# ilovepose/fast-human-pose-estimation.pytorch

Hardware: AMD Instinct MI355X
Metric: images/sec FPD train step (4-stack HG student, 8-stack teacher) 256x256 (higher is better)
Workload: dtype bf16; 1 GPU; configs[1]: hourglass student S=4 F=128 + teacher S=8 F=256, 256x256, batch 32/GPU, fused FPD step incl. Adam, teacher forward one batch ahead on a 2nd stream; global_batch=32, parallelism=dp1, backend=mfma, launch=one native plan call per phase, kernels launched eagerly on 3 streams, ranks=1, finite=True

## Files before the change

### fast-human-pose-estimation.pytorch_amd/csrc/api.hip

```cpp
#include <cstdarg>
#include <cstdio>
#include <cstdlib>
#include <cstring>
#include <string>
#include <vector>

#include "common.h"

int fpd_conv_mfma_launch(const fpd_conv_t& a, hipStream_t st);
int fpd_conv_tile_launch(const fpd_conv_t& a, hipStream_t st);
int fpd_conv_pp_launch(const fpd_conv_t& a, hipStream_t st);
int fpd_conv_c1_launch(const fpd_conv_t& a, hipStream_t st);
int fpd_conv_c3_launch(const fpd_conv_t& a, hipStream_t st);
int fpd_conv_c3_pair_launch(const fpd_conv_t& a, const fpd_conv_t& b, hipStream_t st);
int fpd_conv_c3_fold_ok(const fpd_conv_t& a, const fpd_conv_t* b);
int fpd_conv_c3_option(int which, int value);
int fpd_conv_c1_pair_launch(const fpd_conv_t& a, const fpd_conv_t& b, hipStream_t st);
int fpd_conv_c1_fold_ok(const fpd_conv_t& a, const fpd_conv_t* b);
int fpd_conv_c1_option(int which, int value);
int fpd_conv_c1_wgrad_partials(const fpd_conv_t& a);
int fpd_conv_c1_pair_wgrad_partials(const fpd_conv_t& a, const fpd_conv_t& b, int* na, int* nb);
int fpd_conv_pp_pair_launch(const fpd_conv_t& a, const fpd_conv_t& b, hipStream_t st);
int fpd_conv_pp_fold_ok(const fpd_conv_t& a, const fpd_conv_t* b);
int fpd_conv_tile_fold_ok(const fpd_conv_t& a);
int fpd_conv_tile_pair_fold_ok(const fpd_conv_t& a, const fpd_conv_t& b);
int fpd_conv_pp_option(int which, int value);
int fpd_conv_pp_wgrad_partials(const fpd_conv_t& a);
int fpd_conv_pp_pair_wgrad_partials(const fpd_conv_t& a, const fpd_conv_t& b, int* na, int* nb);
int fpd_conv_tile_pair_launch(const fpd_conv_t& a, const fpd_conv_t& b, hipStream_t st);
int fpd_bneck_fused_launch(const fpd_bneck_t& a, hipStream_t st);
int fpd_bneck_fold_launch(const fpd_bneck_t& a, float* out, hipStream_t st);
int fpd_pck_launch(const fpd_pck_t& a, hipStream_t st);
int fpd_conv_smallc_launch(const fpd_conv_t& a, hipStream_t st);
bool fpd_conv_f8_domain(const fpd_conv_t& a);
int fpd_conv_tile_f8_launch(const fpd_conv_t& a, const void* w8, const float* wscale, hipStream_t st);
int fpd_weight_quant_f8_launch(const fpd_wquant_entry_t* table, int n, hipStream_t st);
int fpd_flip_w_launch(const float* x, float* y, int64_t rows, int W, hipStream_t st);
int fpd_flip_merge_launch(const fpd_flipmerge_t& p, hipStream_t st);
int fpd_final_preds_launch(const fpd_finalpreds_t& p, hipStream_t st);
int fpd_render_targets_launch(const fpd_targets_t& a, hipStream_t st);
int fpd_warp_affine_launch(const fpd_warp_t& a, hipStream_t st);
int fpd_head_fused_launch(const fpd_head_t& a, hipStream_t st);
int fpd_head_fold_launch(const fpd_head_t& a, float* out, hipStream_t st);
int fpd_bneck_fused_pair_launch(const fpd_bneck_t& a, const fpd_bneck_t& b, hipStream_t st);
int fpd_wgrad_mfma_launch(const fpd_wgrad_t& a, hipStream_t st);
int fpd_wgrad_tile_launch(const fpd_wgrad_t& a, hipStream_t st);
int fpd_wgrad_tile_partials(const fpd_wgrad_t& a);
int fpd_wgrad_smallc_launch(const fpd_wgrad_t& a, hipStream_t st);
int fpd_wgrad_smallc_partials(const fpd_wgrad_t& a);
int fpd_wgrad_mfma_partials(const fpd_wgrad_t& a);
int fpd_wgrad_naive_partials(const fpd_wgrad_t& a);
int fpd_stem_wgrad_mfma_partials(const fpd_stem_t& a);
int fpd_stem_wgrad_partials(const fpd_stem_t& a);
int fpd_wreduce_launch(const fpd_wreduce_entry_t* table, int n, int64_t max_elems, hipStream_t st);
int fpd_conv_naive_launch(const fpd_conv_t& a, hipStream_t st);
int fpd_wgrad_naive_launch(const fpd_wgrad_t& a, hipStream_t st);
int fpd_stem_forward_launch(const fpd_stem_t& a, hipStream_t st);
int fpd_stem_forward_mfma_launch(const fpd_stem_t& a, hipStream_t st);
int fpd_stem_forward_s2d_launch(const fpd_stem_t& a, hipStream_t st);
int fpd_stem_wgrad_s2d_launch(const fpd_stem_t& a, hipStream_t st);
int fpd_stem_wgrad_s2d_partials(const fpd_stem_t& a);
int fpd_stem_wgrad_mfma_launch(const fpd_stem_t& a, hipStream_t st);
int fpd_stem_wgrad_launch(const fpd_stem_t& a, hipStream_t st);
int fpd_elementwise_launch(const fpd_ew_t& a, hipStream_t st);
int fpd_elementwise_pair_launch(const fpd_ew_t& a, const fpd_ew_t& b, hipStream_t st);
int fpd_affsum_launch(const fpd_affsum_t& a, hipStream_t st);
int fpd_loss_launch(const fpd_loss_t& a, hipStream_t st);
int fpd_adam_launch(const fpd_adam_t& a, hipStream_t st);
int fpd_weight_prep_launch(const fpd_wprep_entry_t* table, int n, int64_t max_elems, int dtype, hipStream_t st);
int fpd_bn_update_running_launch(const fpd_bnupd_entry_t* table, int n, hipStream_t st);
int fpd_cast_launch(const void* src, void* dst, int64_t n, int sd, int dd, hipStream_t st);
int fpd_nchw_to_nhwc_launch(const float* src, void* dst, int N, int C, int H, int W, int dtype, hipStream_t st);
int fpd_nhwc_to_nchw_launch(const void* src, float* dst, int N, int C, int H, int W, int dtype, hipStream_t st);

int g_fpd_backend = FPD_BACKEND_MFMA;
static thread_local char g_err[512] = "";

static FILE* g_launch_log_file = nullptr;
static bool launch_log_open() {
    const char* path = getenv("FPD_LAUNCH_LOG");
    if (path == nullptr || path[0] == 0) return false;
    g_launch_log_file = fopen(path, "w");
    if (g_launch_log_file == nullptr) fprintf(stderr, "[fpd_amd] FPD_LAUNCH_LOG: cannot open %s\n", path);
    return g_launch_log_file != nullptr;
}
bool g_fpd_launch_log = launch_log_open();
static thread_local char g_op_tag[256] = "-";
void fpd_log_launch(const char* kernel, const dim3& grid, const dim3& block) {
    if (g_launch_log_file == nullptr) return;
    fprintf(g_launch_log_file, "%s\t%u\t%u\t%s\n", kernel, grid.x * grid.y * grid.z, block.x * block.y * block.z, g_op_tag);
    fflush(g_launch_log_file);
}

int fpd_fail(int code, const char* fmt, ...) {
    va_list ap;
    va_start(ap, fmt);
    vsnprintf(g_err, sizeof(g_err), fmt, ap);
    va_end(ap);
    return code;
}

static int check_launch() {
    hipError_t e = hipGetLastError();
    if (e != hipSuccess) return fpd_fail(-100 - (int)e, "kernel launch failed: %s", hipGetErrorString(e));
    return 0;
}

static int validate_conv_dims(int N, int H, int W, int C, int K, int R, int S, int stride, int pad, int P, int Q) {
    FPD_REQUIRE(N > 0 && H > 0 && W > 0 && C > 0 && K > 0 && R > 0 && S > 0 && stride > 0 && pad >= 0,
                "conv: non-positive dimension");
    FPD_REQUIRE(P == (H + 2 * pad - R) / stride + 1 && Q == (W + 2 * pad - S) / stride + 1,
                "conv: output %dx%d inconsistent with input %dx%d k=%dx%d stride=%d pad=%d", P, Q, H, W, R, S, stride, pad);
    FPD_REQUIRE((int64_t)N * H * W * C < (1ll << 31) && (int64_t)N * P * Q * K < (1ll << 31), "conv: tensor too large for 32-bit indexing");
    return 0;
}

extern "C" {

const char* fpd_last_error(void) { return g_err; }
int fpd_abi_version(void) { return FPD_ABI_VERSION; }
int64_t fpd_stats_words(int32_t channels) { return FPD_STATS_WORDS(channels); }
int fpd_set_backend(int32_t backend) {
    const int prev = g_fpd_backend;
    if (backend == FPD_BACKEND_MFMA || backend == FPD_BACKEND_NAIVE || backend == FPD_BACKEND_MFMA_GENERIC) g_fpd_backend = backend;
    return prev;
}

static int g_wgrad_tile_only = 0;

int fpd_set_option(const char* name, int32_t value) {
    FPD_REQUIRE(name, "set_option: null name");
    if (!strcmp(name, "conv_pp")) return fpd_conv_pp_option(0, value);
    if (!strcmp(name, "conv_pp_blocks")) return fpd_conv_pp_option(1, value);
    if (!strcmp(name, "conv_c1")) return fpd_conv_c1_option(0, value);
    if (!strcmp(name, "conv_c1_blocks")) return fpd_conv_c1_option(1, value);
    if (!strcmp(name, "conv_c1_launches")) return fpd_conv_c1_option(2, value);
    if (!strcmp(name, "conv_c3")) return fpd_conv_c3_option(0, value);
    if (!strcmp(name, "conv_c3_blocks")) return fpd_conv_c3_option(1, value);
    if (!strcmp(name, "conv_c3_launches")) return fpd_conv_c3_option(2, value);
    if (!strcmp(name, "wgrad_tile_only")) { g_wgrad_tile_only = value; return 0; }
    return fpd_fail(-2, "set_option: unknown option '%s'", name);
}

int fpd_abi_sizeof(const char* n) {
#define SZ(T) if (!strcmp(n, #T)) return (int)sizeof(T)
    SZ(fpd_bn_t); SZ(fpd_conv_t); SZ(fpd_wgrad_t); SZ(fpd_stem_t); SZ(fpd_ew_t); SZ(fpd_loss_t); SZ(fpd_adam_t);
    SZ(fpd_wprep_entry_t); SZ(fpd_bnupd_entry_t); SZ(fpd_memset_t); SZ(fpd_table_t); SZ(fpd_wreduce_entry_t); SZ(fpd_bneck_t); SZ(fpd_conv_pair_t); SZ(fpd_bneck_pair_t); SZ(fpd_ew_pair_t); SZ(fpd_pck_t); SZ(fpd_head_t); SZ(fpd_affsum_t); SZ(fpd_layout_t);
    SZ(fpd_conv_f8_t); SZ(fpd_wquant_entry_t); SZ(fpd_flipmerge_t); SZ(fpd_finalpreds_t); SZ(fpd_targets_t); SZ(fpd_warp_src_t); SZ(fpd_warp_t);
#undef SZ
    return -1;
}

static int validate_conv(const fpd_conv_t* a) {
    FPD_REQUIRE(a && a->x && a->w && a->y, "conv: null pointer");
    int rc = validate_conv_dims(a->N, a->H, a->W, a->C, a->K, a->R, a->S, a->stride, a->pad, a->P, a->Q);
    if (rc) return rc;
    FPD_REQUIRE(a->dtype == FPD_F32 || a->dtype == FPD_BF16, "conv: bad dtype %d", a->dtype);
    FPD_REQUIRE(a->bn.mode == FPD_BN_NONE || (a->bn.gamma && a->bn.beta), "conv: BN prologue without gamma/beta");
    FPD_REQUIRE(a->bn.mode != FPD_BN_TRAIN || a->bn.stats, "conv: train-mode BN without statistics");
    FPD_REQUIRE(a->bn.mode != FPD_BN_EVAL || (a->bn.running_mean && a->bn.running_var), "conv: eval-mode BN without running stats");
    FPD_REQUIRE(a->epi == FPD_EPI_PLAIN || (a->epi_x && a->epi_stats && a->epi_bn.mode == FPD_BN_TRAIN && a->epi_bn.stats),
                "conv: BNRELU_BWD epilogue needs epi_x, epi_stats and a train-mode epi_bn");
    return 0;
}

static int dispatch_conv(const fpd_conv_t* a, hipStream_t st) {
    int rc = 1;
    if (g_fpd_backend == FPD_BACKEND_MFMA) rc = fpd_conv_c1_launch(*a, st);
    if (rc == 1 && g_fpd_backend == FPD_BACKEND_MFMA) rc = fpd_conv_c3_launch(*a, st);
    if (rc == 1 && g_fpd_backend == FPD_BACKEND_MFMA) rc = fpd_conv_pp_launch(*a, st);
    FPD_REQUIRE(rc != 1 || a->wg_partial == nullptr, "conv: a fused weight gradient (wg_partial) needs the persistent kernel; "
                "fpd_conv_fused_wgrad_partials() reports 0 for this launch");
    if (rc == 1 && g_fpd_backend == FPD_BACKEND_MFMA) rc = fpd_conv_tile_launch(*a, st);
    FPD_REQUIRE(rc != 1 || a->fold_x == nullptr, "conv: a folded BN-backward apply (fold_x) needs the persistent or the halo-tile "
                "kernel; fpd_conv_fold_supported() reports 0 for this launch");
    if (rc == 1 && g_fpd_backend != FPD_BACKEND_NAIVE) rc = fpd_conv_mfma_launch(*a, st);
    if (rc == 1 && g_fpd_backend != FPD_BACKEND_NAIVE) rc = fpd_conv_smallc_launch(*a, st);
    if (rc == 1) rc = fpd_conv_naive_launch(*a, st);
    return rc;
}

int fpd_conv_forward(const fpd_conv_t* a, fpd_stream_t stream) {
    int rc = validate_conv(a);
    if (rc) return rc;
    rc = dispatch_conv(a, (hipStream_t)stream);
    return rc ? rc : check_launch();
}

int fpd_conv_fold_supported(const fpd_conv_t* a) {
    if (!a || g_fpd_backend != FPD_BACKEND_MFMA || validate_conv(a) != 0) return 0;
    return (fpd_conv_c1_fold_ok(*a, nullptr) || fpd_conv_c3_fold_ok(*a, nullptr) || fpd_conv_pp_fold_ok(*a, nullptr) || fpd_conv_tile_fold_ok(*a)) ? 1 : 0;
}
int fpd_conv_pair_fold_supported(const fpd_conv_pair_t* p) {
    if (!p || g_fpd_backend != FPD_BACKEND_MFMA || validate_conv(&p->a) != 0 || validate_conv(&p->b) != 0) return 0;
    if (fpd_conv_c1_fold_ok(p->a, &p->b)) return 1;
    if (fpd_conv_c3_fold_ok(p->a, &p->b)) return 1;
    if (fpd_conv_pp_fold_ok(p->a, &p->b)) return 1;
    const int r = fpd_conv_tile_pair_fold_ok(p->a, p->b);
    if (r >= 0) return r;
    return (fpd_conv_fold_supported(&p->a) && fpd_conv_fold_supported(&p->b)) ? 1 : 0;
}

int fpd_conv_fused_wgrad_partials(const fpd_conv_t* a) {
    if (!a || g_fpd_backend != FPD_BACKEND_MFMA || validate_conv(a) != 0) return 0;
    const int n = fpd_conv_c1_wgrad_partials(*a);
    return n >= 0 ? n : fpd_conv_pp_wgrad_partials(*a);
}
int fpd_conv_pair_fused_wgrad_partials(const fpd_conv_pair_t* p, int32_t* n_a, int32_t* n_b) {
    FPD_REQUIRE(p && n_a && n_b, "conv_pair_fused_wgrad_partials: null pointer");
    *n_a = *n_b = 0;
    if (g_fpd_backend != FPD_BACKEND_MFMA || validate_conv(&p->a) != 0 || validate_conv(&p->b) != 0) return 0;
    int na = 0, nb = 0;
    if (fpd_conv_c1_pair_wgrad_partials(p->a, p->b, &na, &nb) < 0) fpd_conv_pp_pair_wgrad_partials(p->a, p->b, &na, &nb);
    *n_a = na; *n_b = nb;
    return 0;
}

int fpd_conv_f8_in_domain(const fpd_conv_t* c) { return (c && fpd_conv_f8_domain(*c)) ? 1 : 0; }

int fpd_conv_forward_f8(const fpd_conv_f8_t* a, fpd_stream_t stream) {
    FPD_REQUIRE(a, "conv_f8: null pointer");
    int rc = validate_conv(&a->c);
    if (rc) return rc;
    FPD_REQUIRE(a->w8 && a->w8_scale, "conv_f8: null fp8 weights / scales");
    FPD_REQUIRE(((uintptr_t)a->w8 & 15) == 0, "conv_f8: w8 must be 16-byte aligned");
    rc = 1;
    if (g_fpd_backend == FPD_BACKEND_MFMA) rc = fpd_conv_tile_f8_launch(a->c, a->w8, a->w8_scale, (hipStream_t)stream);
    if (rc == 1) rc = dispatch_conv(&a->c, (hipStream_t)stream);
    return rc ? rc : check_launch();
}

int fpd_weight_quant_f8(const fpd_wquant_entry_t* t, int32_t n, fpd_stream_t stream) {
    FPD_REQUIRE(n == 0 || t != nullptr, "weight_quant_f8: null table");
    int rc = fpd_weight_quant_f8_launch(t, n, (hipStream_t)stream);
    return rc ? rc : check_launch();
}

int fpd_conv_forward_pair(const fpd_conv_pair_t* p, fpd_stream_t stream) {
    FPD_REQUIRE(p, "conv_pair: null pointer");
    int rc = validate_conv(&p->a);
    if (rc) return rc;
    rc = validate_conv(&p->b);
    if (rc) return rc;
    hipStream_t st = (hipStream_t)stream;
    rc = 1;
    if (g_fpd_backend == FPD_BACKEND_MFMA) rc = fpd_conv_c1_pair_launch(p->a, p->b, st);
    if (rc == 1 && g_fpd_backend == FPD_BACKEND_MFMA) rc = fpd_conv_c3_pair_launch(p->a, p->b, st);
    if (rc == 1 && g_fpd_backend == FPD_BACKEND_MFMA) rc = fpd_conv_pp_pair_launch(p->a, p->b, st);
    FPD_REQUIRE(rc != 1 || (p->a.wg_partial == nullptr && p->b.wg_partial == nullptr),
                "conv_pair: fused weight gradients need the persistent kernel; fpd_conv_pair_fused_wgrad_partials() reports 0 for this launch");
    if (rc == 1 && g_fpd_backend == FPD_BACKEND_MFMA) rc = fpd_conv_tile_pair_launch(p->a, p->b, st);
    if (rc == 1) {
        rc = dispatch_conv(&p->a, st);
        if (rc == 0) rc = dispatch_conv(&p->b, st);
    }
    return rc ? rc : check_launch();
}

static int validate_bneck_bns(const fpd_bneck_t* a) {
    const fpd_bn_t* bns[3] = {&a->bn1, &a->bn2, &a->bn3};
    for (int i = 0; i < 3; ++i)
        FPD_REQUIRE(bns[i]->mode == FPD_BN_EVAL && bns[i]->relu && bns[i]->gamma && bns[i]->beta && bns[i]->running_mean &&
                    bns[i]->running_var, "bottleneck: bn%d must be an eval-mode BN+ReLU with running statistics", i + 1);
    return 0;
}

int fpd_bottleneck_fold(const fpd_bneck_t* a, fpd_stream_t stream) {
    FPD_REQUIRE(a && a->folded, "bottleneck_fold: null pointer");
    int rc = validate_bneck_bns(a);
    if (rc) return rc;
    rc = fpd_bneck_fold_launch(*a, const_cast<float*>(a->folded), (hipStream_t)stream);
    if (rc == 1) return fpd_fail(-3, "bottleneck_fold: C=%d P=%d is outside the fused kernel's domain", a->C, a->P);
    return rc ? rc : check_launch();
}

int fpd_bottleneck_forward_pair(const fpd_bneck_pair_t* p, fpd_stream_t stream) {
    FPD_REQUIRE(p, "bottleneck_pair: null pointer");
    const fpd_bneck_t* ab[2] = {&p->a, &p->b};
    for (const fpd_bneck_t* a : ab) {
        FPD_REQUIRE(a->x && a->y && a->w1 && a->w2 && a->w3 && a->x != a->y, "bottleneck_pair: null pointer or y aliases x");
        FPD_REQUIRE((int64_t)a->N * a->H * a->W * a->C < ((int64_t)1 << 31), "bottleneck_pair: tensor too large for 32-bit indexing");
        int rc = validate_bneck_bns(a);
        if (rc) return rc;
    }
    int rc = fpd_bneck_fused_pair_launch(p->a, p->b, (hipStream_t)stream);
    if (rc == 1) {
        rc = fpd_bottleneck_forward(&p->a, stream);
        return rc ? rc : fpd_bottleneck_forward(&p->b, stream);
    }
    return rc ? rc : check_launch();
}

// ... 479 lines not shown
```

### fast-human-pose-estimation.pytorch_amd/csrc/bneck_fused.hip

```cpp
#include <algorithm>
#include <cstdlib>
#include <type_traits>

#include "common.h"

namespace {

typedef unsigned int u32x4 __attribute__((ext_vector_type(4)));
template <int N, typename F>
__device__ __forceinline__ void static_for(F&& f) {
    if constexpr (N > 0) {
        static_for<N - 1>(f);
        f(std::integral_constant<int, N - 1>{});
    }
}

#ifdef FPD_BNECK_TIMING
#define STAMP(i) do { if (tid == 0 && bid_in == 0) stamps[i] = clock64(); } while (0)
#else
#define STAMP(i) do { } while (0)
#endif

template <int P>
__device__ __forceinline__ void bneck_fold_tables(const fpd_bneck_t& a, float* out, int tid, int nthreads) {
    constexpr int C = 2 * P;
    for (int c = tid; c < C; c += nthreads) {
        float sc, sh;
        bn_coef_eval(a.bn1, c, sc, sh);
        out[c] = sc;
        out[C + c] = sh;
        out[2 * C + 4 * P + c] = a.b3 ? a.b3[c] : 0.f;
    }
    for (int c = tid; c < 2 * P; c += nthreads) {
        const bool second = c >= P;
        const int cc = second ? c - P : c;
        float sc, sh;
        bn_coef_eval(second ? a.bn3 : a.bn2, cc, sc, sh);
        const float* bias = second ? a.b2 : a.b1;
        out[2 * C + (second ? 2 * P : 0) + cc] = sc;
        out[2 * C + (second ? 2 * P : 0) + P + cc] = fmaf(sc, bias ? bias[cc] : 0.f, sh);
    }
}

template <int P>
__global__ void bneck_fold_kernel(const fpd_bneck_t a, float* out) { bneck_fold_tables<P>(a, out, threadIdx.x, blockDim.x); }

template <int P, bool DMA>
__device__ __forceinline__ void bneck_eval_body(const fpd_bneck_t& a, const int logW, const int swz, const int bid_in,
                                                const int nblk, const int ntiles) {
    constexpr int C = 2 * P;
    constexpr int LDW = DMA ? P : P + 8;
    constexpr int LDX = 64 + 8;
    constexpr int LD2 = P + 8;
    constexpr int TNH = P / 64;
    constexpr int CW = 32 * TNH;
    constexpr int NSTEP = 9 + 2;
    constexpr int VPR2 = P / 8;
    constexpr int WV = P * VPR2 / 512;
    constexpr int W1V = P * 8 / 512;
    constexpr int NCH = C / 64;
    constexpr int ASTG = (128 + P) * LDX;
    extern __shared__ __attribute__((aligned(16))) unsigned char smem[];

    const int tid = threadIdx.x, lane = tid & 63, wave = tid >> 6;
#ifdef FPD_BNECK_TIMING
    long long stamps[8];
    long long astamp[10];
    int acnt = 0;
#define ASTAMP() do { if (tid == 0 && bid_in == 0 && acnt < 10) astamp[acnt++] = clock64(); } while (0)
#else
#define ASTAMP() do { } while (0)
#endif
    STAMP(0);
    const int q = wave & 3, hC = wave >> 2;
    const int koff = 8 * (lane >> 5);
    const int H = a.H, W = a.W;
    const int M = a.N * H * W, GR = a.N * H;
    const int nrows = 128 >> logW, hrows = nrows + 2, WP = W + 2;
    const int rrows = 2 * nrows;
    const bool whole = (128 % (H * W)) == 0;
    const int irows = whole ? hrows : rrows;
    const int zero_px = irows * WP;
    int m0 = 0, g0 = 0;
    int vrow0 = 0;

    float* s_sc1 = reinterpret_cast<float*>(smem);
    float* s_sh1 = s_sc1 + C;
    float* s_sc2 = s_sh1 + C;
    float* s_sh2 = s_sc2 + P;
    float* s_sc3 = s_sh2 + P;
    float* s_sh3 = s_sc3 + P;
    float* s_b3 = s_sh3 + P;
    bf16_t* sA2 = reinterpret_cast<bf16_t*>(s_b3 + C);
    bf16_t* sR2 = sA2 + (zero_px + 3) * LD2;
    const bf16_t* __restrict__ x = reinterpret_cast<const bf16_t*>(a.x);
    const bf16_t* __restrict__ w1 = reinterpret_cast<const bf16_t*>(a.w1);
    const bf16_t* __restrict__ w2 = reinterpret_cast<const bf16_t*>(a.w2);
    const bf16_t* __restrict__ w3 = reinterpret_cast<const bf16_t*>(a.w3);

    int hp0 = whole ? W : 0;
    int npass = whole ? 1 : ((hrows * W + 127) >> 7);
    const int xpx = tid >> 3, xcv = (tid & 7) * 8;
    int xo[2];
    bool xok[2];
    auto pass_addr = [&](int p) __attribute__((always_inline)) {
#pragma unroll
        for (int i = 0; i < 2; ++i) {
            const int hp = hp0 + 128 * p + xpx + 64 * i;
            const int hr = hp >> logW, j = hp & (W - 1);
            const int g = g0 - 1 + hr;
            xok[i] = hr < hrows && (unsigned)g < (unsigned)GR;
            xo[i] = xok[i] ? (g * W + j) * C + xcv : 0;
        }
    };
    int w1o[W1V], w1l[W1V];
#pragma unroll
    for (int i = 0; i < W1V; ++i) {
        const int v = tid + i * 512;
        w1o[i] = (v >> 3) * C + (v & 7) * 8;
        w1l[i] = 128 * LDX + (v >> 3) * LDX + (v & 7) * 8;
    }
    const int xl = xpx * LDX + xcv;

    u32x4 rx[NCH][2], rw[NCH][W1V];
    auto a_load = [&](auto kcc) __attribute__((always_inline)) {
        constexpr int kc = decltype(kcc)::value;
        static_for<2>([&](auto ic) {
            constexpr int i = decltype(ic)::value;
            const u32x4 z = {0u, 0u, 0u, 0u};
            rx[kc][i] = z;
            if (xok[i]) rx[kc][i] = *reinterpret_cast<const u32x4*>(x + (xo[i] + kc * 64));
        });
        static_for<W1V>([&](auto ic) {
            constexpr int i = decltype(ic)::value;
            rw[kc][i] = *reinterpret_cast<const u32x4*>(w1 + (w1o[i] + kc * 64));
        });
    };
    constexpr int NSL = 2 + W1V;
    auto a_store_slice = [&](auto kcc, auto slc) __attribute__((always_inline)) {
        constexpr int kc = decltype(kcc)::value, sl = decltype(slc)::value;
        bf16_t* dst = sR2 + (kc & 1) * ASTG;
        if constexpr (sl < 2) {
            f32x4 sc[2], sh[2];
            sc[0] = *reinterpret_cast<const f32x4*>(s_sc1 + kc * 64 + xcv);
            sc[1] = *reinterpret_cast<const f32x4*>(s_sc1 + kc * 64 + xcv + 4);
            sh[0] = *reinterpret_cast<const f32x4*>(s_sh1 + kc * 64 + xcv);
            sh[1] = *reinterpret_cast<const f32x4*>(s_sh1 + kc * 64 + xcv + 4);
            float f[8];
            const u32x4 r = rx[kc][sl];
            DT<bf16_t>::unpack(make_uint4(r[0], r[1], r[2], r[3]), f);
#pragma unroll
            for (int e = 0; e < 8; ++e) f[e] = fmaxf(fmaf(f[e], sc[e >> 2][e & 3], sh[e >> 2][e & 3]), 0.f);
            *reinterpret_cast<uint4*>(dst + xl + 64 * sl * LDX) = DT<bf16_t>::pack(f);
        } else if constexpr (sl < NSL) {
            *reinterpret_cast<u32x4*>(dst + w1l[sl - 2]) = rw[kc][sl - 2];
        }
    };
    auto a_store = [&](auto kcc) __attribute__((always_inline)) {
        static_for<NSL>([&](auto slc) { a_store_slice(kcc, slc); });
    };
    int t2o[WV], t3o[WV], tlo[WV];
#pragma unroll
    for (int i = 0; i < WV; ++i) {
        const int v = tid + i * 512;
        const int row = v / VPR2, col = (v - row * VPR2) * 8;
        t2o[i] = row * 9 * P + col;
        t3o[i] = row * P + col;
        tlo[i] = row * LD2 + col;
    }
    u32x4 rb[DMA ? 1 : 2][DMA ? 1 : WV];
    auto t_load = [&](auto sc_) __attribute__((always_inline)) {
        constexpr int s = decltype(sc_)::value;
        if constexpr (!DMA) {
            static_for<WV>([&](auto ic) {
                constexpr int i = decltype(ic)::value;
                const bf16_t* src = s < 9 ? w2 + (t2o[i] + s * P) : w3 + (t3o[i] + (s - 9) * P * P);
                rb[s & 1][i] = *reinterpret_cast<const u32x4*>(src);
            });
        }
    };
    auto t_store = [&](auto sc_) __attribute__((always_inline)) {
        constexpr int s = decltype(sc_)::value;
        if constexpr (!DMA) {
            bf16_t* dst = sR2 + (s & 1) * P * LDW;
            static_for<WV>([&](auto ic) {
                constexpr int i = decltype(ic)::value;
                *reinterpret_cast<u32x4*>(dst + tlo[i]) = rb[s & 1][i];
            });
        }
    };
    constexpr int CPR = P / 8;
    constexpr int RPI = 64 / CPR;
    constexpr int DPW = P / RPI / 8;
    unsigned dma2[DMA ? DPW : 1], dma3[DMA ? DPW : 1];
    if constexpr (DMA) {
// ... 211 lines not shown
        if constexpr (s == 8) {
            STAMP(4);
            bf16_t* dst = sA2 + (a3px + ml) * LD2;
#pragma unroll
            for (int tn = 0; tn < TNH; ++tn)
#pragma unroll
                for (int gi = 0; gi < 4; ++gi) {
                    const int c = hC * CW + tn * 32 + 8 * gi + 4 * (lane >> 5);
                    const f32x4 sc = *reinterpret_cast<const f32x4*>(s_sc3 + c);
                    const f32x4 sh = *reinterpret_cast<const f32x4*>(s_sh3 + c);
                    float v[4];
#pragma unroll
                    for (int e = 0; e < 4; ++e) v[e] = fmaxf(fmaf(accB[tn][4 * gi + e], sc[e], sh[e]), 0.f);
                    *reinterpret_cast<uint2*>(dst + c) = make_uint2(f2bf_pk(v[0], v[1]), f2bf_pk(v[2], v[3]));
                }
            __syncthreads();
        }
    });

    STAMP(5);
    constexpr int LDS_ = CW + 4;
    float* stage = reinterpret_cast<float*>(sR2) + wave * 32 * LDS_;
    bf16_t* __restrict__ y = reinterpret_cast<bf16_t*>(a.y);
    static_for<2>([&](auto stc) {
        constexpr int st = decltype(stc)::value;
        __syncthreads();
#pragma unroll
        for (int tn = 0; tn < TNH; ++tn)
#pragma unroll
            for (int gi = 0; gi < 4; ++gi) {
                f32x4 v;
#pragma unroll
                for (int e = 0; e < 4; ++e) v[e] = accC[st][tn][4 * gi + e];
                *reinterpret_cast<f32x4*>(stage + (lane & 31) * LDS_ + tn * 32 + 8 * gi + 4 * (lane >> 5)) = v;
            }
        __syncthreads();
        static_for<NIT>([&](auto itc) {
            constexpr int it = decltype(itc)::value;
            const int idx = lane + 64 * it;
            const int px = idx / VW, cv = (idx - px * VW) * 8;
            const int m = m0 + q * 32 + px;
            if (m < M) {
                const int c = st * P + hC * CW + cv;
                const f32x4 v0 = *reinterpret_cast<const f32x4*>(stage + px * LDS_ + cv);
                const f32x4 v1 = *reinterpret_cast<const f32x4*>(stage + px * LDS_ + cv + 4);
                const f32x4 b0 = *reinterpret_cast<const f32x4*>(s_b3 + c);
                const f32x4 b1 = *reinterpret_cast<const f32x4*>(s_b3 + c + 4);
                float res[8], o[8];
                const u32x4 r = rres[st][it];
                DT<bf16_t>::unpack(make_uint4(r[0], r[1], r[2], r[3]), res);
#pragma unroll
                for (int e = 0; e < 4; ++e) {
                    o[e] = v0[e] + b0[e] + res[e];
                    o[4 + e] = v1[e] + b1[e] + res[4 + e];
                }
                *reinterpret_cast<uint4*>(y + ((size_t)m * C + c)) = DT<bf16_t>::pack(o);
            }
        });
    });
    }
#ifdef FPD_BNECK_TIMING
    STAMP(6);
    if (tid == 0 && bid_in == 0)
        printf("bneck W=%d: setup %lld | phaseA %lld | tile0 %lld | B(9 taps) %lld | a3+C %lld | epilogue %lld | total %lld cycles\n",
               W, stamps[1] - stamps[0], stamps[2] - stamps[1], stamps[3] - stamps[2], stamps[4] - stamps[3],
               stamps[5] - stamps[4], stamps[6] - stamps[5], stamps[6] - stamps[0]);
    if (tid == 0 && bid_in == 0 && acnt == 10)
        printf("  phase A steps: first-stage %lld | pass0 %lld %lld %lld %lld | pass1 %lld %lld %lld %lld | a2 write %lld\n",
               astamp[1] - astamp[0], astamp[2] - astamp[1], astamp[3] - astamp[2], astamp[4] - astamp[3], astamp[5] - astamp[4],
               astamp[6] - astamp[5], astamp[7] - astamp[6], astamp[8] - astamp[7], astamp[9] - astamp[8], stamps[2] - astamp[9]);
#endif
}

template <int P, bool DMA>
__global__ __launch_bounds__(512, 1) void bneck_eval_kernel(const fpd_bneck_t a, const int logW, const int ntiles) {
    bneck_eval_body<P, DMA>(a, logW, (ntiles & 7) == 0, blockIdx.x, gridDim.x, ntiles);
}

template <int P, bool DMA>
__global__ __launch_bounds__(512, 1) void bneck_eval_pair_kernel(const fpd_bneck_t a, const fpd_bneck_t b, const int logWa,
                                                                 const int logWb, const int nblk_a, const int ntiles_a,
                                                                 const int ntiles_b) {
    if ((int)blockIdx.x < nblk_a) bneck_eval_body<P, DMA>(a, logWa, (ntiles_a & 7) == 0, blockIdx.x, nblk_a, ntiles_a);
    else bneck_eval_body<P, DMA>(b, logWb, (ntiles_b & 7) == 0, (int)blockIdx.x - nblk_a, (int)gridDim.x - nblk_a, ntiles_b);
}


static int bneck_block_cap() {
    static int cap = 0;
    if (!cap) {
        const char* e = getenv("FPD_BNECK_BLOCKS");
        cap = e ? atoi(e) : 128;
        if (cap < 8) cap = 8;
    }
    return cap;
}
static int bneck_blocks(int tiles, int cap) {
    if (tiles <= cap) return tiles;
    const int rounds = cdiv(tiles, cap);
    return cdiv(tiles, rounds);
}

template <int P>
size_t bneck_lds_bytes(int H, int W) {
    constexpr int C = 2 * P, LD2 = P + 8, LDX = 72, CW = 32 * (P / 64);
    int logW = 0;
    while ((1 << logW) < W) ++logW;
    const int nrows = 128 >> logW, WP = W + 2;
    const bool whole = (128 % (H * W)) == 0;
    const int irows = whole ? nrows + 2 : 2 * nrows;
    const size_t r2 = std::max({(size_t)2 * P * LD2 * 2, (size_t)2 * (128 + P) * LDX * 2, (size_t)8 * 32 * (CW + 4) * 4});
    return (size_t)(3 * C + 4 * P) * sizeof(float) + (size_t)(irows * WP + 3) * LD2 * 2 + r2;
}

template <int P, bool DMA>
int launch_bneck_pair(const fpd_bneck_t& a, const fpd_bneck_t& b, hipStream_t st) {
    const size_t lds = std::max(bneck_lds_bytes<P>(a.H, a.W), bneck_lds_bytes<P>(b.H, b.W));
    static LdsAttr configured;
    if (int rc_ = configured.ensure(reinterpret_cast<const void*>(&bneck_eval_pair_kernel<P, DMA>), lds)) return rc_;
    int la = 0, lb = 0;
    while ((1 << la) < a.W) ++la;
    while ((1 << lb) < b.W) ++lb;
    const int ta = cdiv(a.N * a.H * a.W, 128), tb = cdiv(b.N * b.H * b.W, 128);
    int na = ta, nb = tb;
    const int cap = bneck_block_cap();
    if (ta + tb > cap) {
        const int capb = std::max(1, (int)((int64_t)cap * tb / (ta + tb)));
        nb = bneck_blocks(tb, capb);
        na = bneck_blocks(ta, std::max(1, cap - nb));
    }
    FPD_LAUNCH((bneck_eval_pair_kernel<P, DMA>), dim3(na + nb), dim3(512), lds, st, a, b, la, lb, na, ta, tb);
    return 0;
}

template <int P, bool DMA>
int launch_bneck(const fpd_bneck_t& a, int logW, hipStream_t st) {
    const size_t lds = bneck_lds_bytes<P>(a.H, a.W);
    static LdsAttr configured;
    if (int rc_ = configured.ensure(reinterpret_cast<const void*>(&bneck_eval_kernel<P, DMA>), lds)) return rc_;
    const int ntiles = cdiv(a.N * a.H * a.W, 128);
    FPD_LAUNCH((bneck_eval_kernel<P, DMA>), dim3(bneck_blocks(ntiles, bneck_block_cap())), dim3(512), lds, st, a, logW, ntiles);
    return 0;
}

}

static bool bneck_in_domain(const fpd_bneck_t& a) {
    if (a.dtype != FPD_BF16 || a.C != 2 * a.P || (a.P != 64 && a.P != 128)) return false;
    if (a.W < 4 || a.W > 64 || (a.W & (a.W - 1)) != 0) return false;
    const int hw = a.H * a.W;
    return hw % 128 == 0 || 128 % hw == 0;
}

int fpd_bneck_fused_launch(const fpd_bneck_t& a, hipStream_t st) {
    if (!bneck_in_domain(a)) return 1;
    int logW = 0;
    while ((1 << logW) < a.W) ++logW;
    return a.P == 128 ? launch_bneck<128, true>(a, logW, st) : launch_bneck<64, true>(a, logW, st);
}

int fpd_bneck_fused_pair_launch(const fpd_bneck_t& a, const fpd_bneck_t& b, hipStream_t st) {
    if (!bneck_in_domain(a) || !bneck_in_domain(b) || a.P != b.P) return 1;
    return a.P == 128 ? launch_bneck_pair<128, true>(a, b, st) : launch_bneck_pair<64, true>(a, b, st);
}

int fpd_bneck_fold_launch(const fpd_bneck_t& a, float* out, hipStream_t st) {
    if (a.C != 2 * a.P || (a.P != 64 && a.P != 128)) return 1;
    if (a.P == 128) FPD_LAUNCH((bneck_fold_kernel<128>), dim3(1), dim3(256), 0, st, a, out);
    else FPD_LAUNCH((bneck_fold_kernel<64>), dim3(1), dim3(256), 0, st, a, out);
    return 0;
}
```

Before: 3687 images/s.

## Add wide-tile fused bottleneck kernel for P=128 at W=32/64

Adds a new fused bottleneck kernel for P=128, C=256 layers at 32- or 64-wide resolutions. Each 512-thread block processes 256-pixel tiles and reuses the conv1 halo rows incrementally across consecutive tiles. It streams the conv2/conv3 weights into LDS with global_load_lds double buffering and stages the residual epilogue through LDS. The intent is to cut redundant halo recompute and weight reloads compared with the 128-pixel tile kernel, at the cost of one block per CU (launch_bounds 512,1) and large LDS use, which limits occupancy. It is enabled by default and falls back to the old path outside its domain.

Measured after the change: 3691 images/s, median of 6. No clear change (+0.1%).

```diff
diff --git a/fast-human-pose-estimation.pytorch_amd/csrc/api.hip b/fast-human-pose-estimation.pytorch_amd/csrc/api.hip
--- a/fast-human-pose-estimation.pytorch_amd/csrc/api.hip
+++ b/fast-human-pose-estimation.pytorch_amd/csrc/api.hip
@@ -43,6 +43,7 @@
 int fpd_head_fused_launch(const fpd_head_t& a, hipStream_t st);
 int fpd_head_fold_launch(const fpd_head_t& a, float* out, hipStream_t st);
 int fpd_bneck_fused_pair_launch(const fpd_bneck_t& a, const fpd_bneck_t& b, hipStream_t st);
+int fpd_bneck_wide_option(int which, int value);
 int fpd_wgrad_mfma_launch(const fpd_wgrad_t& a, hipStream_t st);
 int fpd_wgrad_tile_launch(const fpd_wgrad_t& a, hipStream_t st);
 int fpd_wgrad_tile_partials(const fpd_wgrad_t& a);
@@ -138,6 +139,9 @@
     if (!strcmp(name, "conv_c3")) return fpd_conv_c3_option(0, value);
     if (!strcmp(name, "conv_c3_blocks")) return fpd_conv_c3_option(1, value);
     if (!strcmp(name, "conv_c3_launches")) return fpd_conv_c3_option(2, value);
+    if (!strcmp(name, "bneck_wide")) return fpd_bneck_wide_option(0, value);
+    if (!strcmp(name, "bneck_wide_blocks")) return fpd_bneck_wide_option(1, value);
+    if (!strcmp(name, "bneck_wide_launches")) return fpd_bneck_wide_option(2, value);
     if (!strcmp(name, "wgrad_tile_only")) { g_wgrad_tile_only = value; return 0; }
     return fpd_fail(-2, "set_option: unknown option '%s'", name);
 }
diff --git a/fast-human-pose-estimation.pytorch_amd/csrc/bneck_fused.hip b/fast-human-pose-estimation.pytorch_amd/csrc/bneck_fused.hip
--- a/fast-human-pose-estimation.pytorch_amd/csrc/bneck_fused.hip
+++ b/fast-human-pose-estimation.pytorch_amd/csrc/bneck_fused.hip
@@ -2,6 +2,7 @@
 #include <cstdlib>
 #include <type_traits>
 
+#include "bneck_tables.h"
 #include "common.h"
 
 namespace {
@@ -20,27 +21,6 @@
 #else
 #define STAMP(i) do { } while (0)
 #endif
-
-template <int P>
-__device__ __forceinline__ void bneck_fold_tables(const fpd_bneck_t& a, float* out, int tid, int nthreads) {
-    constexpr int C = 2 * P;
-    for (int c = tid; c < C; c += nthreads) {
-        float sc, sh;
-        bn_coef_eval(a.bn1, c, sc, sh);
-        out[c] = sc;
-        out[C + c] = sh;
-        out[2 * C + 4 * P + c] = a.b3 ? a.b3[c] : 0.f;
-    }
-    for (int c = tid; c < 2 * P; c += nthreads) {
-        const bool second = c >= P;
-        const int cc = second ? c - P : c;
-        float sc, sh;
-        bn_coef_eval(second ? a.bn3 : a.bn2, cc, sc, sh);
-        const float* bias = second ? a.b2 : a.b1;
-        out[2 * C + (second ? 2 * P : 0) + cc] = sc;
-        out[2 * C + (second ? 2 * P : 0) + P + cc] = fmaf(sc, bias ? bias[cc] : 0.f, sh);
-    }
-}
 
 template <int P>
 __global__ void bneck_fold_kernel(const fpd_bneck_t a, float* out) { bneck_fold_tables<P>(a, out, threadIdx.x, blockDim.x); }
@@ -558,7 +538,11 @@
     return hw % 128 == 0 || 128 % hw == 0;
 }
 
+int fpd_bneck_wide_launch(const fpd_bneck_t& a, hipStream_t st);
+int fpd_bneck_wide_pair_launch(const fpd_bneck_t& a, const fpd_bneck_t& b, hipStream_t st);
+
 int fpd_bneck_fused_launch(const fpd_bneck_t& a, hipStream_t st) {
+    if (int rc = fpd_bneck_wide_launch(a, st); rc != 1) return rc;
     if (!bneck_in_domain(a)) return 1;
     int logW = 0;
     while ((1 << logW) < a.W) ++logW;
@@ -566,6 +550,7 @@
 }
 
 int fpd_bneck_fused_pair_launch(const fpd_bneck_t& a, const fpd_bneck_t& b, hipStream_t st) {
+    if (int rc = fpd_bneck_wide_pair_launch(a, b, st); rc != 1) return rc;
     if (!bneck_in_domain(a) || !bneck_in_domain(b) || a.P != b.P) return 1;
     return a.P == 128 ? launch_bneck_pair<128, true>(a, b, st) : launch_bneck_pair<64, true>(a, b, st);
 }
diff --git a/fast-human-pose-estimation.pytorch_amd/csrc/bneck_tables.h b/fast-human-pose-estimation.pytorch_amd/csrc/bneck_tables.h
--- /dev/null
+++ b/fast-human-pose-estimation.pytorch_amd/csrc/bneck_tables.h
@@ -0,0 +1,23 @@
+#pragma once
+#include "common.h"
+
+template <int P>
+__device__ __forceinline__ void bneck_fold_tables(const fpd_bneck_t& a, float* out, int tid, int nthreads) {
+    constexpr int C = 2 * P;
+    for (int c = tid; c < C; c += nthreads) {
+        float sc, sh;
+        bn_coef_eval(a.bn1, c, sc, sh);
+        out[c] = sc;
+        out[C + c] = sh;
+        out[2 * C + 4 * P + c] = a.b3 ? a.b3[c] : 0.f;
+    }
+    for (int c = tid; c < 2 * P; c += nthreads) {
+        const bool second = c >= P;
+        const int cc = second ? c - P : c;
+        float sc, sh;
+        bn_coef_eval(second ? a.bn3 : a.bn2, cc, sc, sh);
+        const float* bias = second ? a.b2 : a.b1;
+        out[2 * C + (second ? 2 * P : 0) + cc] = sc;
+        out[2 * C + (second ? 2 * P : 0) + P + cc] = fmaf(sc, bias ? bias[cc] : 0.f, sh);
+    }
+}
diff --git a/fast-human-pose-estimation.pytorch_amd/csrc/bneck_wide.hip b/fast-human-pose-estimation.pytorch_amd/csrc/bneck_wide.hip
--- /dev/null
+++ b/fast-human-pose-estimation.pytorch_amd/csrc/bneck_wide.hip
@@ -0,0 +1,477 @@
+#include <algorithm>
+#include <atomic>
+#include <cstdlib>
+#include <type_traits>
+
+#include "bneck_tables.h"
+#include "common.h"
+
+namespace {
+
+typedef unsigned int u32x4 __attribute__((ext_vector_type(4)));
+
+template <int N, typename F>
+__device__ __forceinline__ void static_for(F&& f) {
+    if constexpr (N > 0) {
+        static_for<N - 1>(f);
+        f(std::integral_constant<int, N - 1>{});
+    }
+}
+template <int V>
+using ic_t = std::integral_constant<int, V>;
+
+constexpr int WP_ = 128, WC_ = 256;
+constexpr int TPX = 256;
+constexpr int LD2 = WP_ + 8;
+constexpr int NTAB = 3 * WC_ + 4 * WP_;
+constexpr int RBYTES = 49152;
+constexpr int SLOT = 16384;
+constexpr int XS = 32;
+constexpr int STG = (TPX + WP_) * XS;
+constexpr int LDE = 64 + 8;
+constexpr int NH = 22;
+static_assert(2 * STG * 2 <= RBYTES && 2 * SLOT <= RBYTES && 8 * 32 * LDE * 2 <= RBYTES, "region R");
+
+__device__ __forceinline__ void wave_lds_sync() {
+    asm volatile("s_waitcnt lgkmcnt(0)" ::: "memory");
+    __builtin_amdgcn_wave_barrier();
+}
+
+#ifdef FPD_BNECK_TIMING
+#define WSTAMP(i) do { if (tid == 0 && bid_in == 0) stamps[i] = clock64(); } while (0)
+#else
+#define WSTAMP(i) do { } while (0)
+#endif
+
+__device__ __forceinline__ void bneck_wide_body(const fpd_bneck_t& a, const int logW, const int bid_in, const int nblk,
+                                                const int ntiles) {
+    constexpr int P = WP_, C = WC_;
+    extern __shared__ __attribute__((aligned(16))) unsigned char smem[];
+    const int tid = threadIdx.x, lane = tid & 63, wave = tid >> 6;
+#ifdef FPD_BNECK_TIMING
+    long long stamps[8] = {0, 0, 0, 0, 0, 0, 0, 0};
+#endif
+    WSTAMP(0);
+    const int q = wave & 3, hC = wave >> 2, hi = lane >> 5, l32 = lane & 31;
+    const int H = a.H, W = a.W, GR = a.N * H;
+    const int nrows = TPX >> logW, hrows = nrows + 2, RR = nrows + 2, WP = W + 2;
+    const int zero_px = RR * WP;
+
+    float* s_sc1 = reinterpret_cast<float*>(smem);
+    float* s_sh1 = s_sc1 + C;
+    float* s_sc2 = s_sh1 + C;
+    float* s_sh2 = s_sc2 + P;
+    float* s_sc3 = s_sh2 + P;
+    float* s_sh3 = s_sc3 + P;
+    float* s_b3 = s_sh3 + P;
+    unsigned char* sR = smem + NTAB * 4;
+    bf16_t* sRb = reinterpret_cast<bf16_t*>(sR);
+    bf16_t* sA2 = reinterpret_cast<bf16_t*>(sR + RBYTES);
+    const bf16_t* __restrict__ x = reinterpret_cast<const bf16_t*>(a.x);
+    const bf16_t* __restrict__ w1 = reinterpret_cast<const bf16_t*>(a.w1);
+    const bf16_t* __restrict__ w2 = reinterpret_cast<const bf16_t*>(a.w2);
+    const bf16_t* __restrict__ w3 = reinterpret_cast<const bf16_t*>(a.w3);
+    bf16_t* __restrict__ y = reinterpret_cast<bf16_t*>(a.y);
+
+    if (a.folded != nullptr) {
+        for (int v = tid; v < NTAB / 4; v += 512)
+            reinterpret_cast<f32x4*>(s_sc1)[v] = reinterpret_cast<const f32x4*>(a.folded)[v];
+    } else {
+        bneck_fold_tables<P>(a, s_sc1, tid, 512);
+    }
+    {
+        constexpr int VR = LD2 / 8;
+        const uint4 z = make_uint4(0, 0, 0, 0);
+        for (int v = tid; v < (2 * RR + 3) * VR; v += 512) {
+            const int pz = v / VR, cv = (v - pz * VR) * 8;
+            const int px = pz < 2 * RR ? ((pz >> 1) * WP + ((pz & 1) ? WP - 1 : 0)) : zero_px + (pz - 2 * RR);
+            *reinterpret_cast<uint4*>(sA2 + px * LD2 + cv) = z;
+        }
+    }
+
+    const int xp = tid >> 2, xc = tid & 3;
+    const int stl = xp * XS + ((xc ^ ((xp >> 2) & 3)) * 8);
+    const int w1o = xp * C + xc * 8;
+    int hp0 = 0, npass = 2, g0 = 0;
+    int xo[2];
+    bool xok[2];
+    auto pass_addr = [&](int p) __attribute__((always_inline)) {
+#pragma unroll
+        for (int i = 0; i < 2; ++i) {
+            const int hp = hp0 + TPX * p + xp + 128 * i;
+            const int hr = hp >> logW, j = hp & (W - 1);
+            const int g = g0 - 1 + hr;
+            xok[i] = hr < hrows && (unsigned)g < (unsigned)GR;
+            xo[i] = xok[i] ? (g * W + j) * C + xc * 8 : 0;
+        }
+    };
+    u32x4 rx[8][2], rw[8];
+    auto a_load = [&](auto kcc) __attribute__((always_inline)) {
+        constexpr int kc = decltype(kcc)::value;
+        static_for<2>([&](auto ic) {
+            constexpr int i = decltype(ic)::value;
+            const u32x4 z = {0u, 0u, 0u, 0u};
+            rx[kc][i] = z;
+            if (xok[i]) rx[kc][i] = *reinterpret_cast<const u32x4*>(x + (xo[i] + kc * XS));
+        });
+        rw[kc] = *reinterpret_cast<const u32x4*>(w1 + (w1o + kc * XS));
+    };
+    auto a_store_slice = [&](auto kcc, auto slc) __attribute__((always_inline)) {
+        constexpr int kc = decltype(kcc)::value, sl = decltype(slc)::value;
+        bf16_t* dst = sRb + (kc & 1) * STG;
+        if constexpr (sl < 2) {
+            const int c0 = kc * XS + xc * 8;
+            const f32x4 sc0 = *reinterpret_cast<const f32x4*>(s_sc1 + c0), sc1 = *reinterpret_cast<const f32x4*>(s_sc1 + c0 + 4);
+            const f32x4 sh0 = *reinterpret_cast<const f32x4*>(s_sh1 + c0), sh1 = *reinterpret_cast<const f32x4*>(s_sh1 + c0 + 4);
+            float f[8];
+            const u32x4 r = rx[kc][sl];
+            DT<bf16_t>::unpack(make_uint4(r[0], r[1], r[2], r[3]), f);
+#pragma unroll
+            for (int e = 0; e < 4; ++e) {
+                f[e] = fmaxf(fmaf(f[e], sc0[e], sh0[e]), 0.f);
+                f[4 + e] = fmaxf(fmaf(f[4 + e], sc1[e], sh1[e]), 0.f);
+            }
+            *reinterpret_cast<uint4*>(dst + stl + sl * 128 * XS) = DT<bf16_t>::pack(f);
+        } else {
+            *reinterpret_cast<u32x4*>(dst + TPX * XS + stl) = rw[kc];
+        }
+    };
+    const int xsw = (lane >> 2) & 3;
+    const int c1o0 = ((0 + hi) ^ xsw) * 8, c1o1 = ((2 + hi) ^ xsw) * 8;
+
+    unsigned dma2[2], dma3[2];
+#pragma unroll
+    for (int j = 0; j < 2; ++j) {
+        const int row = (wave * 2 + j) * 8 + (lane >> 3);
+        const int c8 = ((lane & 7) ^ ((row >> 1) & 7)) * 8;
+        dma2[j] = (unsigned)(row * 9 * P + c8) * 2u;
+        dma3[j] = (unsigned)(row * P + c8) * 2u;
+    }
+    auto t_dma = [&](auto hc_) __attribute__((always_inline)) {
+        constexpr int h = decltype(hc_)::value;
+        unsigned char* slot = sR + (h & 1) * SLOT + wave * 2 * 1024;
+        const char* gbase = h < 18 ? reinterpret_cast<const char*>(w2) + ((h >> 1) * P + (h & 1) * 64) * 2
+                                   : reinterpret_cast<const char*>(w3) + (((h - 18) >> 1) * P * P + (h & 1) * 64) * 2;
+        static_for<2>([&](auto jc) {
+            constexpr int j = decltype(jc)::value;
+            unsigned off = h < 18 ? dma2[j] : dma3[j];
+            asm volatile("" : "+v"(off));
+            __builtin_amdgcn_global_load_lds((const __attribute__((address_space(1))) void*)(gbase + off),
+                                             (__attribute__((address_space(3))) void*)(slot + j * 1024), 16, 0, 0);
+        });
+    };
+    const int wsw = (lane >> 1) & 7;
+    int wko[4];
+#pragma unroll
+    for (int kk = 0; kk < 4; ++kk) wko[kk] = ((2 * kk + hi) ^ wsw) * 8;
+
+    const int t_beg = fpd_cut(bid_in, ntiles, nblk), t_end = fpd_cut(bid_in + 1, ntiles, nblk);
+    for (int tile = t_beg; tile < t_end; ++tile) {
+        g0 = tile * nrows;
+        const bool incr = tile > t_beg && (g0 % H) != 0;
+        hp0 = incr ? 2 * W : 0;
+        npass = incr ? 1 : 2;
+        pass_addr(0);
+        static_for<8>([&](auto kcc) { a_load(kcc); });
+        if (npass > 1) pass_addr(1);
+        __syncthreads();
+        WSTAMP(1);
+
+        static_for<3>([&](auto slc) { a_store_slice(ic_t<0>{}, slc); });
+        if (npass > 1) a_load(ic_t<0>{});
+        __syncthreads();
+        for (int p = 0; p < npass; ++p) {
+            f32x16 acc[2][2];
+            static_for<2>([&](auto pmc) {
+                static_for<2>([&](auto tnc) {
+#pragma unroll
+                    for (int i = 0; i < 16; ++i) acc[pmc][tnc][i] = 0.f;
+                });
+            });
+            static_for<8>([&](auto kcc) {
+                constexpr int kc = decltype(kcc)::value;
+                auto stage_slice = [&](auto slc) __attribute__((always_inline)) {
+                    constexpr int sl = decltype(slc)::value;
+                    if constexpr (kc + 1 < 8) {
+                        a_store_slice(ic_t<kc + 1>{}, slc);
+                        if constexpr (sl == 2) {
+                            if (p + 1 < npass) a_load(ic_t<kc + 1>{});
+                        }
+                    } else {
+                        if (p + 1 < npass) a_store_slice(ic_t<0>{}, slc);
+                    }
+                };
+                const bf16_t* xb = sRb + (kc & 1) * STG + (q * 64 + l32) * XS;
+                const bf16_t* wb = sRb + (kc & 1) * STG + TPX * XS + (hC * 64 + l32) * XS;
+                static_for<2>([&](auto kkc) {
+                    constexpr int kk = decltype(kkc)::value;
+                    const int co = kk ? c1o1 : c1o0;
+                    bf16x8 px[2], wf[2];
+                    static_for<2>([&](auto ic) {
+                        constexpr int i = decltype(ic)::value;
+                        px[i] = *reinterpret_cast<const bf16x8*>(xb + i * 32 * XS + co);
+                        wf[i] = *reinterpret_cast<const bf16x8*>(wb + i * 32 * XS + co);
+                    });
+                    static_for<2>([&](auto pmc) {
+                        static_for<2>([&](auto tnc) {
+                            acc[pmc][tnc] = __builtin_amdgcn_mfma_f32_32x32x16_bf16(wf[tnc], px[pmc], acc[pmc][tnc], 0, 0, 0);
+                        });
+                    });
+                    if constexpr (kk == 0) {
+                        stage_slice(ic_t<0>{});
+                        stage_slice(ic_t<1>{});
+                    } else {
+                        stage_slice(ic_t<2>{});
+                    }
+                });
+                __syncthreads();
+            });
+            if (p + 1 == npass) {
+                t_dma(ic_t<0>{});
+                t_dma(ic_t<1>{});
+            }
+            static_for<2>([&](auto pmc) {
+                constexpr int pm = decltype(pmc)::value;
+                const int hp = hp0 + TPX * p + q * 64 + pm * 32 + l32;
+                const int hr = hp >> logW, j = hp & (W - 1);
+                if (hr < hrows) {
+                    bf16_t* dst = sA2 + (((g0 + hr) % RR) * WP + j + 1) * LD2;
+                    static_for<2>([&](auto tnc) {
+                        constexpr int tn = decltype(tnc)::value;
+#pragma unroll
+                        for (int gi = 0; gi < 4; ++gi) {
+                            const int c = hC * 64 + tn * 32 + 8 * gi + 4 * hi;
+                            const f32x4 sc = *reinterpret_cast<const f32x4*>(s_sc2 + c);
+                            const f32x4 sh = *reinterpret_cast<const f32x4*>(s_sh2 + c);
+                            float v[4];
+#pragma unroll
+                            for (int e = 0; e < 4; ++e) v[e] = fmaxf(fmaf(acc[pm][tn][4 * gi + e], sc[e], sh[e]), 0.f);
+                            *reinterpret_cast<uint2*>(dst + c) = make_uint2(f2bf_pk(v[0], v[1]), f2bf_pk(v[2], v[3]));
+                        }
+                    });
+                }
+            });
+        }
+
+        int ab[2][3], a3o[2];
+        static_for<2>([&](auto pmc) {
+            constexpr int pm = decltype(pmc)::value;
+            const int ml = q * 64 + pm * 32 + l32;
+            const int ti = ml >> logW, tj = ml & (W - 1);
+            const int pr = (g0 + ti) % H;
+            const int r0 = (g0 + ti) % RR, r1 = (g0 + ti + 1) % RR, r2 = (g0 + ti + 2) % RR;
+            ab[pm][0] = pr - 1 >= 0 ? (r0 * WP + tj) * LD2 : zero_px * LD2;
+            ab[pm][1] = (r1 * WP + tj) * LD2;
+            ab[pm][2] = pr + 1 < H ? (r2 * WP + tj) * LD2 : zero_px * LD2;
+            a3o[pm] = (r0 * WP + tj + 1) * LD2;
+        });
+        WSTAMP(2);
+        __syncthreads();
+        WSTAMP(3);
+
+        f32x16 accB[2][2], accC[2][2][2];
+        static_for<2>([&](auto pmc) {
+            static_for<2>([&](auto tnc) {
+#pragma unroll
+                for (int i = 0; i < 16; ++i) accB[pmc][tnc][i] = 0.f;
+            });
+        });
+        const bf16_t* wrow = sRb + (hC * 64 + l32) * 64;
+        auto mma = [&](const bf16_t* a0, const bf16_t* a1, int buf, f32x16 (&acc)[2][2]) __attribute__((always_inline)) {
+            const bf16_t* wb = wrow + buf * (SLOT / 2);
+            static_for<4>([&](auto kkc) {
+                constexpr int kk = decltype(kkc)::value;
+                bf16x8 px[2], wf[2];
+                px[0] = *reinterpret_cast<const bf16x8*>(a0 + kk * 16);
+                px[1] = *reinterpret_cast<const bf16x8*>(a1 + kk * 16);
+                wf[0] = *reinterpret_cast<const bf16x8*>(wb + wko[kk]);
+                wf[1] = *reinterpret_cast<const bf16x8*>(wb + 32 * 64 + wko[kk]);
+                static_for<2>([&](auto pmc) {
+                    static_for<2>([&](auto tnc) {
+                        acc[pmc][tnc] = __builtin_amdgcn_mfma_f32_32x32x16_bf16(wf[tnc], px[pmc], acc[pmc][tnc], 0, 0, 0);
+                    });
+                });
+            });
+        };
+
+        u32x4 rres[2][4];
+        const int m0 = g0 * W;
+        auto res_load = [&](auto rc_) __attribute__((always_inline)) {
+            constexpr int r = decltype(rc_)::value, st = r >> 1, pm = r & 1;
+            static_for<4>([&](auto itc) {
+                constexpr int it = decltype(itc)::value;
+                const int idx = lane + 64 * it;
+                const int px = idx >> 3, cv = (idx & 7) * 8;
+                const int m = m0 + q * 64 + pm * 32 + px;
+                rres[r & 1][it] = *reinterpret_cast<const u32x4*>(x + ((size_t)m * C + st * P + hC * 64 + cv));
+            });
+        };
+
+        static_for<NH>([&](auto hc_) {
+            constexpr int h = decltype(hc_)::value;
+            if constexpr (h >= 1 && h + 1 < NH) t_dma(ic_t<(h + 1 < NH ? h + 1 : 0)>{});
+            if constexpr (h < 18) {
+                constexpr int s = h >> 1, dr = s / 3, dc = s % 3, ko = (h & 1) * 64;
+                mma(sA2 + ab[0][dr] + dc * LD2 + ko + 8 * hi, sA2 + ab[1][dr] + dc * LD2 + ko + 8 * hi, h & 1, accB);
+            } else {
+                constexpr int st = (h - 18) >> 1, ko = (h & 1) * 64;
+                if constexpr ((h & 1) == 0) {
+                    static_for<2>([&](auto pmc) {
+                        static_for<2>([&](auto tnc) {
+#pragma unroll
+                            for (int i = 0; i < 16; ++i) accC[st][pmc][tnc][i] = 0.f;
+                        });
+                    });
+                }
+                mma(sA2 + a3o[0] + ko + 8 * hi, sA2 + a3o[1] + ko + 8 * hi, h & 1, accC[st]);
+            }
+            if constexpr (h == 20) res_load(ic_t<0>{});
+            if constexpr (h + 1 < NH) __syncthreads();
+            if constexpr (h == 17) {
+                WSTAMP(4);
+                static_for<2>([&](auto pmc) {
+                    constexpr int pm = decltype(pmc)::value;
+                    bf16_t* dst = sA2 + a3o[pm];
+                    static_for<2>([&](auto tnc) {
+                        constexpr int tn = decltype(tnc)::value;
+#pragma unroll
+                        for (int gi = 0; gi < 4; ++gi) {
+                            const int c = hC * 64 + tn * 32 + 8 * gi + 4 * hi;
+                            const f32x4 sc = *reinterpret_cast<const f32x4*>(s_sc3 + c);
+                            const f32x4 sh = *reinterpret_cast<const f32x4*>(s_sh3 + c);
+                            float v[4];
+#pragma unroll
+                            for (int e = 0; e < 4; ++e) v[e] = fmaxf(fmaf(accB[pm][tn][4 * gi + e], sc[e], sh[e]), 0.f);
+                            *reinterpret_cast<uint2*>(dst + c) = make_uint2(f2bf_pk(v[0], v[1]), f2bf_pk(v[2], v[3]));
+                        }
+                    });
+                });
+                __syncthreads();
+            }
+        });
+        WSTAMP(5);
+
+        __syncthreads();
+        bf16_t* stage = sRb + wave * 32 * LDE;
+        static_for<4>([&](auto rc_) {
+            constexpr int r = decltype(rc_)::value, st = r >> 1, pm = r & 1;
+            static_for<4>([&](auto itc) {
+                constexpr int it = decltype(itc)::value;
+                const int idx = lane + 64 * it;
+                *reinterpret_cast<u32x4*>(stage + (idx >> 3) * LDE + (idx & 7) * 8) = rres[r & 1][it];
+            });
+            if constexpr (r + 1 < 4) res_load(ic_t<(r + 1 < 4 ? r + 1 : 0)>{});
+            wave_lds_sync();
+            static_for<2>([&](auto tnc) {
+                constexpr int tn = decltype(tnc)::value;
+#pragma unroll
+                for (int gi = 0; gi < 4; ++gi) {
+                    const int c = tn * 32 + 8 * gi + 4 * hi;
+                    uint2* sp = reinterpret_cast<uint2*>(stage + l32 * LDE + c);
+                    const uint2 rv = *sp;
+                    const f32x4 b = *reinterpret_cast<const f32x4*>(s_b3 + st * P + hC * 64 + c);
+                    const float res[4] = {__uint_as_float(rv.x << 16), __uint_as_float(rv.x & 0xffff0000u),
+                                          __uint_as_float(rv.y << 16), __uint_as_float(rv.y & 0xffff0000u)};
+                    float o[4];
+#pragma unroll
+                    for (int e = 0; e < 4; ++e) o[e] = accC[st][pm][tn][4 * gi + e] + b[e] + res[e];
+                    *sp = make_uint2(f2bf_pk(o[0], o[1]), f2bf_pk(o[2], o[3]));
+                }
+            });
+            wave_lds_sync();
+            static_for<4>([&](auto itc) {
+                constexpr int it = decltype(itc)::value;
+                const int idx = lane + 64 * it;
+                const int px = idx >> 3, cv = (idx & 7) * 8;
+                const int m = m0 + q * 64 + pm * 32 + px;
+                *reinterpret_cast<uint4*>(y + ((size_t)m * C + st * P + hC * 64 + cv)) =
+                    *reinterpret_cast<const uint4*>(stage + px * LDE + cv);
+            });
+            wave_lds_sync();
+        });
+    }
+#ifdef FPD_BNECK_TIMING
+    WSTAMP(6);
+    if (tid == 0 && bid_in == 0)
+        printf("bneck_wide W=%d (last tile): setup+loads %lld | conv1 %lld | a2 barrier %lld | conv2 (18 half-steps) %lld | a3+conv3 %lld"
+               " | epilogue %lld cycles\n", W, stamps[1] - stamps[0], stamps[2] - stamps[1], stamps[3] - stamps[2],
+               stamps[4] - stamps[3], stamps[5] - stamps[4], stamps[6] - stamps[5]);
+#endif
+}
+
+__global__ __launch_bounds__(512, 1) void bneck_wide_kernel(const fpd_bneck_t a, const int logW, const int ntiles) {
+    bneck_wide_body(a, logW, blockIdx.x, gridDim.x, ntiles);
+}
+
+__global__ __launch_bounds__(512, 1) void bneck_wide_pair_kernel(const fpd_bneck_t a, const fpd_bneck_t b, const int logWa,
+                                                                 const int logWb, const int nblk_a, const int ntiles_a,
+                                                                 const int ntiles_b) {
+    if ((int)blockIdx.x < nblk_a) bneck_wide_body(a, logWa, blockIdx.x, nblk_a, ntiles_a);
+    else bneck_wide_body(b, logWb, (int)blockIdx.x - nblk_a, (int)gridDim.x - nblk_a, ntiles_b);
+}
+
+int g_wide_mode = -1, g_wide_blocks = -1;
+std::atomic<int> g_wide_launches{0};
+int wide_mode() {
+    if (g_wide_mode < 0) { const char* e = getenv("FPD_BNECK_WIDE"); g_wide_mode = e ? atoi(e) : 1; }
+    return g_wide_mode;
+}
+int wide_blocks() {
+    if (g_wide_blocks < 0) { const char* e = getenv("FPD_BNECK_WIDE_BLOCKS"); g_wide_blocks = e ? atoi(e) : 128; }
+    return std::max(g_wide_blocks, 8);
+}
+int wide_grid(int tiles, int cap) {
+    if (tiles <= cap) return tiles;
+    return cdiv(tiles, cdiv(tiles, cap));
+}
+bool wide_domain(const fpd_bneck_t& a) {
+    return a.dtype == FPD_BF16 && a.P == WP_ && a.C == WC_ && (a.W == 32 || a.W == 64) && (a.H * a.W) % TPX == 0;
+}
+int log2i(int v) {
+    int l = 0;
+    while ((1 << l) < v) ++l;
+    return l;
+}
+size_t wide_lds_bytes(int W) {
+    const int RR = TPX / W + 2;
+    return (size_t)NTAB * 4 + RBYTES + (size_t)(RR * (W + 2) + 3) * LD2 * 2;
+}
+
+}
+
+int fpd_bneck_wide_option(int which, int value) {
+    if (which == 2) return g_wide_launches.load(std::memory_order_relaxed);
+    int& g = which == 0 ? g_wide_mode : g_wide_blocks;
+    const int prev = which == 0 ? wide_mode() : wide_blocks();
+    g = value;
+    return prev;
+}
+
+int fpd_bneck_wide_launch(const fpd_bneck_t& a, hipStream_t st) {
+    if (!wide_mode() || !wide_domain(a)) return 1;
+    const size_t lds = wide_lds_bytes(a.W);
+    static LdsAttr configured;
+    if (int rc_ = configured.ensure(reinterpret_cast<const void*>(&bneck_wide_kernel), lds)) return rc_;
+    const int ntiles = a.N * a.H * a.W / TPX;
+    FPD_LAUNCH(bneck_wide_kernel, dim3(wide_grid(ntiles, wide_blocks())), dim3(512), lds, st, a, log2i(a.W), ntiles);
+    g_wide_launches.fetch_add(1, std::memory_order_relaxed);
+    return 0;
+}
+
+int fpd_bneck_wide_pair_launch(const fpd_bneck_t& a, const fpd_bneck_t& b, hipStream_t st) {
+    if (!wide_mode() || !wide_domain(a) || !wide_domain(b)) return 1;
+    const size_t lds = std::max(wide_lds_bytes(a.W), wide_lds_bytes(b.W));
+    static LdsAttr configured;
+    if (int rc_ = configured.ensure(reinterpret_cast<const void*>(&bneck_wide_pair_kernel), lds)) return rc_;
+    const int ta = a.N * a.H * a.W / TPX, tb = b.N * b.H * b.W / TPX;
+    int na = ta, nb = tb;
+    const int cap = wide_blocks();
+    if (ta + tb > cap) {
+        const int capb = std::max(1, (int)((int64_t)cap * tb / (ta + tb)));
+        nb = wide_grid(tb, capb);
+        na = wide_grid(ta, std::max(1, cap - nb));
+    }
+    FPD_LAUNCH(bneck_wide_pair_kernel, dim3(na + nb), dim3(512), lds, st, a, b, log2i(a.W), log2i(b.W), na, ta, tb);
+    g_wide_launches.fetch_add(1, std::memory_order_relaxed);
+    return 0;
+}
```
